# mic-rud/Learned-Compression-of-Point-Cloud-Geometry-and-Attributes

Hardware: AMD Instinct MI355X
Metric: encode+decode Mpoints/sec (higher is better)
Workload: dtype f32

## Files before the change

### include/pcc_hip.h

```cpp
#ifndef PCC_HIP_H
#define PCC_HIP_H

#include <stdint.h>

#ifdef __cplusplus
extern "C" {
#endif

#define PCC_OK 0
#define PCC_ERR_ARG (-1)
#define PCC_ERR_HIP (-2)
#define PCC_ERR_UNSUPPORTED (-3)
#define PCC_ERR_DATA (-4)

#define PCC_ACT_NONE 0
#define PCC_ACT_RELU 1
#define PCC_ACT_LEAKY_RELU 2

int pcc_version(void);
const char* pcc_last_error(void);
int pcc_device_count(void);
int pcc_device_name(int dev, char* out, int out_len);

int64_t pcc_hash_capacity(int64_t n);
// ... 40 lines not shown
int pcc_pair_count(const uint32_t* row_mask, int64_t n_out, int64_t* pair_count, void* stream);

int64_t pcc_order_scratch_bytes(int64_t n);
int pcc_order_rows_by_mask(const uint32_t* row_mask, const int32_t* coords, int64_t n,
                           int32_t block_log2, int32_t tensor_stride, int32_t* order, uint32_t* group_mask32,
                           void* scratch, int64_t scratch_bytes, void* stream);
int pcc_permute_map_rows(const int32_t* nbr, const int32_t* order, int64_t n, int32_t K, int32_t* nbr_sorted, void* stream);

int64_t pcc_small_map_max(void);
int32_t pcc_small_paths(int32_t mask);
int pcc_small_kernel_map(const int32_t* out_coords, int64_t n_out, const uint64_t* in_keys, const int32_t* in_vals, int64_t in_cap,
                         int32_t ksize, int32_t step, int32_t sign, int32_t* nbr, uint32_t* row_mask, int32_t* order,
                         uint32_t* group_mask32, void* scratch, int64_t scratch_bytes, void* stream);

int64_t pcc_conv_packed_elems(int32_t K, int32_t cin, int32_t cout);
int pcc_conv_pack_weights(const float* w, int32_t K, int32_t cin, int32_t cout, float* w_packed,
                          void* stream);
int pcc_conv_fwd(const float* fin, int64_t n_in, int32_t cin, const float* w, const float* w_packed,
                 const float* bias, const int32_t* nbr, const int32_t* order,
                 const uint32_t* group_mask32, int32_t K, float* fout, int64_t n_out, int32_t cout,
                 int32_t act, const float* film, const float* residual, void* stream);

int64_t pcc_conv_small_max(int64_t workgroups);

int pcc_conv_kernel_name(int32_t mode, int64_t n_in, int32_t cin, int32_t cout, int64_t n_out, int32_t K, int32_t has_nbr,
                         char* buf, int32_t len);

int64_t pcc_conv_packed_elems_bf16(int32_t K, int32_t cin, int32_t cout);
int pcc_conv_pack_weights_bf16(const float* w, int32_t K, int32_t cin, int32_t cout, uint16_t* w_packed, void* stream);
int pcc_conv_fwd_bf16(const uint16_t* fin, int64_t n_in, int32_t cin, const uint16_t* w_packed, const float* bias,
                      const int32_t* nbr, const int32_t* order, const uint32_t* group_mask32, int32_t K, float* fout,
                      int64_t n_out, int32_t cout, int32_t act, const float* film, const float* residual, void* stream);

int pcc_epilogue_fwd(const float* c, const float* film, const float* residual, int64_t n, int32_t channels, int32_t act,
                     float* out, void* stream);
int pcc_epilogue_bwd(const float* dout, const float* c, const float* film, int64_t n, int32_t channels, int32_t act,
                     float* dc, float* dfilm, void* stream);

int64_t pcc_cast_colsum_scratch_elems(int32_t channels);
int pcc_cast_colsum(const float* x, int64_t n, int32_t channels, uint16_t* out_bf16, float* colsum, float* scratch,
                    int64_t scratch_elems, void* stream);

int64_t pcc_conv_packed_elems_x3(int32_t K, int32_t cin, int32_t cout);
int pcc_conv_pack_weights_x3(const float* w, int32_t K, int32_t cin, int32_t cout, uint16_t* w_packed, void* stream);
int pcc_conv_fwd_x3(const float* fin, int64_t n_in, int32_t cin, const uint16_t* w_packed, const float* bias,
                    const int32_t* nbr, const int32_t* order, const uint32_t* group_mask32, int32_t K, float* fout,
                    int64_t n_out, int32_t cout, int32_t act, const float* film, const float* residual, void* stream);

int pcc_im2col_thin(const float* fin, int32_t cin, const int32_t* nbr, int64_t n_out, int32_t K, float* out, int32_t k2,
                    void* stream);

int pcc_gather_sum_fwd(const float* scores, int32_t ld, const int32_t* nbr, int32_t K, int32_t cout,
                       const float* bias, float* out, int64_t n_out, int32_t act, void* stream);

int pcc_gather_rows(const float* src, int32_t c, const int32_t* idx, int64_t n, float* out,
                    int32_t accumulate, void* stream);

int pcc_scatter_rows(const float* src, int32_t c, const int32_t* idx, int64_t n, float* out,
                     void* stream);
int pcc_scatter_add_rows(const float* src, int32_t c, const int32_t* idx, int64_t n, float* out,
                         void* stream);

int pcc_compact_rows(const uint8_t* mask, int64_t n, const int32_t* coords, int32_t* out_coords,
                     const float* feats, int32_t c, float* out_feats, int32_t* new_index,
                     int32_t* scratch, int64_t* out_count, void* stream);

int64_t pcc_topk_state_elems(int32_t nbatch);
int pcc_topk_mask(const float* logits, int32_t ld, const int32_t* coords, int64_t n, int32_t nbatch,
                  const int32_t* k, uint8_t* mask, int32_t* state, void* stream);

int pcc_count_per_batch(const int32_t* coords, int64_t n, int32_t nbatch, int32_t* counts, void* stream);

int64_t pcc_sort_scratch_bytes(int64_t n);
int pcc_sort_coords(const int32_t* coords, int64_t n, int32_t* perm, void* scratch,
                    int64_t scratch_bytes, void* stream);

int pcc_kernel_map_transpose(const int32_t* nbr, int64_t n_out, int32_t K, int64_t n_in, int32_t* nbr_t,
                             uint32_t* row_mask_t, void* stream);
int64_t pcc_conv_wgrad_scratch_elems(int32_t K, int32_t cin, int32_t cout);
int pcc_conv_wgrad(const float* fin, int64_t n_in, int32_t cin, const float* dy, int64_t n_out, int32_t cout,
                   const int32_t* nbr, const int32_t* order, const uint32_t* group_mask32, int32_t K, float* dw,
                   float* scratch, int64_t scratch_elems, void* stream);
int pcc_conv_wgrad_kernel_name(int32_t bf16, int32_t K, int32_t cin, int32_t cout, int64_t n_out, char* buf, int32_t len,
                               int32_t* split, int32_t* partials);
int pcc_conv_wgrad_bf16(const uint16_t* fin, int64_t n_in, int32_t cin, const uint16_t* dy, int64_t n_out, int32_t cout,
                        const int32_t* nbr, const int32_t* order, const uint32_t* group_mask32, int32_t K, float* dw,
                        float* scratch, int64_t scratch_elems, void* stream);

int pcc_chconv(const float* x, int64_t n, int32_t c, const int32_t* coords, const uint64_t* keys, const int32_t* vals,
               int64_t cap, int32_t tensor_stride, int32_t ksize, const float* w, int32_t w_channels, int32_t flip,
               float* y, void* stream);

int64_t pcc_octree_scratch_bytes(int64_t n);
int pcc_octree_occupancy(const int32_t* coords, int64_t n, int32_t stride, const int32_t* origin,
                         int32_t depth, uint8_t* occupancy, int32_t* level_counts, void* scratch,
                         int64_t scratch_bytes, void* stream);
int pcc_octree_expand(const uint8_t* occupancy, const int64_t* level_counts, int32_t depth,
                      int32_t stride, const int32_t* origin, int32_t batch, int64_t n_points,
                      int32_t* coords_out, void* scratch, int64_t scratch_bytes, void* stream);

int pcc_octree_context_levels(const int32_t* coords, int64_t n, int32_t stride, const int32_t* origin,
                              int32_t depth, uint8_t* occupancy, uint8_t* patterns, uint32_t* hists,
                              int32_t* level_counts, void* scratch, int64_t scratch_bytes, void* stream);
int pcc_octree_patterns(const uint64_t* nodes, int64_t n, int32_t level, uint8_t* patterns, void* stream);
int pcc_octree_expand_level(const uint64_t* nodes, const uint8_t* occupancy, int64_t n, int64_t n_next,
                            uint64_t* next, void* scratch, int64_t scratch_bytes, void* stream);
// ... 121 lines not shown
```

### learned-compression-of-point-cloud-geometry-and-attributes_amd/_build.py

```python
import os
import subprocess

_HERE = os.path.dirname(os.path.abspath(__file__))
SO_PATH = os.path.join(_HERE, "libpcc_hip.so")

NO_SCRATCH = {
    "conv": ("conv_small_kernel", "conv_mfma_buf_kernel", "conv_mfma_kernel"),
    "rans_lanes": ("rans_lanes_encode_kernel", "rans_lanes_pack_kernel", "rans_lanes_decode_kernel"),
    "chconv": ("chconv_kernel",),
    "augment": ("jitter_partial_kernel", "jitter_mean_kernel", "jitter_apply_kernel", "first_rows_clear_kernel",
                "first_rows_insert_kernel", "first_rows_flag_kernel", "first_rows_finalize_kernel"),
    "normals": ("estimate_normals_kernel",),
    "voxelize": ("first_rows_clear_kernel", "first_rows_insert_kernel", "first_rows_flag_kernel", "first_rows_finalize_kernel",
                 "voxelize_accumulate_kernel"),
    "raht": ("raht_plan_kernel", "raht_step_kernel", "raht_fold_kernel"),
    "pcqm": ("surface_variation_kernel", "pcqm_features_kernel"),
    "render": ("splat_kernel", "gather_kernel"),
}


def build(force=False):
    args = ["make", "-s", "-C", os.path.join(_HERE, "csrc"), "-j4"]
    if force:
        subprocess.check_call(args + ["clean"])
    subprocess.check_call(args)
    for stem, kernels in NO_SCRATCH.items():
        check_kernel_resources(os.path.join(_HERE, "build", stem + ".resources.txt"), kernels)
    check_small_kernel_lds_reads()
    return SO_PATH


def check_small_kernel_lds_reads(obj=None):
    import glob
    import shutil
    objdump = "/opt/rocm/lib/llvm/bin/llvm-objdump"
    obj = obj or os.path.join(_HERE, "build", "conv.o")
    if not os.path.exists(objdump) or not os.path.exists(obj):
        raise RuntimeError(f"cannot lint conv_small_kernel: {objdump} or {obj} is missing")
    tmp = os.path.join(_HERE, "build", "_lint")
    shutil.rmtree(tmp, ignore_errors=True)
    os.makedirs(tmp)
    local = os.path.join(tmp, "conv.o")
    shutil.copy(obj, local)
    subprocess.run([objdump, "--offloading", local], check=True, capture_output=True, cwd=tmp)
    cos = [f for f in glob.glob(local + ".*") if "amdgcn" in f]
    if not cos:
        raise RuntimeError("cannot lint conv_small_kernel: no device code object in build/conv.o")
    dis = subprocess.run([objdump, "-d", cos[0]], check=True, capture_output=True, text=True).stdout
    shutil.rmtree(tmp, ignore_errors=True)
    return lint_lds_reads(dis)


def lint_lds_reads(dis, kernel="conv_small_kernel"):
    import re

    def regs(operand):
        m = re.fullmatch(r"v\[(\d+):(\d+)\]", operand)
        if m:
            return set(range(int(m.group(1)), int(m.group(2)) + 1))
        m = re.fullmatch(r"v(\d+)", operand)
# ... 67 lines not shown
```

### learned-compression-of-point-cloud-geometry-and-attributes_amd/csrc/conv.hip

```cpp
#include <stdlib.h>

#include <type_traits>

#include "common.h"

namespace pcc {

typedef float f32x2 __attribute__((ext_vector_type(2)));
typedef float f32x4 __attribute__((ext_vector_type(4)));
typedef __bf16 bf16x8 __attribute__((ext_vector_type(8)));

struct ConvArgs {
    const float* fin;
    const float* w;
    const float* wp;
    const float* bias;
    const int32_t* nbr;
    const int32_t* order;
    const uint32_t* gmask;
    float* fout;
    const float* film;
    const float* residual;
    int64_t n_in, n_out;
    int cin, cout, coutp, K, act;
// ... 305 lines not shown
        for_live_pattern<MT>(live_tiles(mmask, k), [&](auto live_tag) {
            mfma_step<decltype(live_tag)::value, BN, false>(acc, a_addr, w_addr);
        });
    };

    if (tmask != 0u) {
        uint32_t rem = tmask;
        int k = __builtin_ctz(rem);
        rem &= rem - 1u;
        int knext = rem ? __builtin_ctz(rem) : -1;
        load_idx(k, idx_cur);
        set_a_src(idx_cur);
        dma_step(k, 0, 0);
        load_idx(knext >= 0 ? knext : k, idx_nxt);
        __syncthreads();
        int c = 0, cur = 0;
        while (true) {
            int nk = k, nc = c + 1;
            if (nc == CCH) { nc = 0; nk = knext; }
            const bool has_next = nk >= 0;
            const bool advance = (nc == 0);
            if (advance) {
#pragma unroll
                for (int i = 0; i < RPT; ++i) idx_cur[i] = idx_nxt[i];
                set_a_src(idx_cur);
            }
            if (has_next) {
                dma_step(nk, nc, cur ^ 1);
            }
            uint32_t rem2 = rem;
            int kn2 = knext;
            if (advance) { rem2 &= rem2 - 1u; kn2 = rem2 ? __builtin_ctz(rem2) : -1; }
            load_idx(kn2 >= 0 ? kn2 : k, idx_nxt);
            compute(cur, k);
            __syncthreads();
            if (!has_next) break;
            if (advance) { k = nk; rem = rem2; knext = kn2; }
            c = nc;
            cur ^= 1;
        }
    }

    conv_store_tiles(a, acc, row0 + wrow, nt * BN + wcol + r, h);
}

template <int I, int N, class F>
__device__ __forceinline__ void static_for(F&& f) {
    if constexpr (I < N) {
        f(std::integral_constant<int, I>{});
        static_for<I + 1, N>(f);
    }
}

template <int BM, int BN, int WAVES_M, int WAVES_N, int CCH, bool HAS_NBR, bool BF16 = false, bool X3 = false>
__global__ __launch_bounds__(256) void conv_mfma_buf_kernel(const ConvArgs a) {
#if defined(__HIP_DEVICE_COMPILE__)
    constexpr int RPT = BM / 32;
    constexpr int WM = BM / WAVES_M, WN = BN / WAVES_N;
    constexpr int MT = WM / 32, NT = WN / 32;
    constexpr int A_ELEMS = BM * 32;
    constexpr int W_ELEMS = (X3 ? 12 : 8) * BN * 4;
    constexpr int W_LOADS = ((X3 ? 12 : 8) * BN) / 256;
    static_assert(WAVES_M * WAVES_N == 4 && MT >= 1 && MT <= 2 && NT >= 1 && W_LOADS >= 1, "bad tiling");
    static_assert(!(BF16 && X3), "one operand mode at a time");
    constexpr int ESZ = BF16 ? 2 : 4;

    extern __shared__ __attribute__((aligned(16))) float smem[];
    float* As = smem;
    float* Ws = smem + 2 * A_ELEMS;

    const int t = threadIdx.x;
    const int lane = t & 63, wid = t >> 6;
    const int r = lane & 31, h = lane >> 5;
    const int wrow = (wid / WAVES_N) * WM, wcol = (wid % WAVES_N) * WN;

    const int ntiles_n = a.coutp / BN;
    const int64_t tile = blockIdx.x / ntiles_n;
    const int nt = blockIdx.x - (int)(tile * ntiles_n);
    const int64_t row0 = tile * BM;
    const int K = a.K;

    uint32_t mmask[MT];
    const uint32_t tmask = conv_live_offsets<BM>(a, row0, wrow, mmask);

    f32x16 acc[MT][NT] = {};

    if (tmask != 0u) {
        __amdgpu_buffer_rsrc_t rsrc_a = __builtin_amdgcn_make_buffer_rsrc(
            const_cast<float*>(a.fin), 0, (int)(uint32_t)(a.n_in * a.cin * ESZ), BUF_FLAGS);
        __amdgpu_buffer_rsrc_t rsrc_w = __builtin_amdgcn_make_buffer_rsrc(
            const_cast<float*>(a.wp), 0, (int)((uint32_t)K * a.cin * a.coutp * (X3 ? 6 : ESZ)), BUF_FLAGS);
        __amdgpu_buffer_rsrc_t rsrc_n = __builtin_amdgcn_make_buffer_rsrc(
            const_cast<int32_t*>(a.nbr), 0, HAS_NBR ? (int)(uint32_t)(a.n_out * K * 4) : 0, BUF_FLAGS);

        const int gchunk = t & 7;
        uint32_t q16[RPT], n_voff[RPT], a_voff[RPT];
        int idx_nxt[RPT];
        bool rvalid[RPT];
#pragma unroll
        for (int i = 0; i < RPT; ++i) {
            const int grow = wid * (BM / 4) + 8 * i + (lane >> 3);
            const int64_t pos = row0 + grow;
            rvalid[i] = pos < a.n_out;
            const int64_t ps = rvalid[i] ? pos : a.n_out - 1;
            q16[i] = (uint32_t)((gchunk ^ ((grow >> 1) & 7)) * 16);
            n_voff[i] = (uint32_t)(((HAS_NBR && a.order) ? (int64_t)a.order[ps] : ps) * K * 4);
            idx_nxt[i] = (int)ps;
        }
// ... 107 lines not shown
                PCC_X3_TERM(ah, bh);
#undef PCC_X3_TERM
            }
            __builtin_amdgcn_s_setprio(0);
        };
        auto compute = [&](auto bufc, unsigned live) {
            for_live_pattern<MT>(live, [&](auto live_tag) {
                if constexpr (X3) compute_live_x3(bufc, live_tag);
                else mfma_step<decltype(live_tag)::value, BN, BF16>(acc, a_addr[decltype(bufc)::value], w_addr[decltype(bufc)::value]);
            });
        };

        uint32_t rem = tmask;
        int k = __builtin_ctz(rem);
        rem &= rem - 1u;
        auto offset_body = [&](auto pc) {
            constexpr int P = decltype(pc)::value;
            const int knext = rem ? __builtin_ctz(rem) : -1;
            const uint32_t rem2 = rem & (rem - 1u);
            const int kn2 = rem2 ? __builtin_ctz(rem2) : (knext >= 0 ? knext : k);
            const unsigned live = live_tiles(mmask, k);
            static_for<0, CCH>([&](auto cc) {
                constexpr int c = decltype(cc)::value;
                constexpr int buf = (P + c) & 1;
                if constexpr (c + 1 < CCH) {
                    dma(k, std::integral_constant<int, c + 1>{}, std::integral_constant<int, buf ^ 1>{});
                } else {
                    set_src(knext >= 0);
                    dma(knext >= 0 ? knext : k, std::integral_constant<int, 0>{}, std::integral_constant<int, buf ^ 1>{});
                    load_idx(kn2);
                }
                compute(std::integral_constant<int, buf>{}, live);
                __syncthreads();
            });
            const bool more = knext >= 0;
            k = more ? knext : k;
            rem = rem2;
            return more;
        };

        load_idx(k);
        set_src(true);
        dma(k, std::integral_constant<int, 0>{}, std::integral_constant<int, 0>{});
        load_idx(rem ? __builtin_ctz(rem) : k);
        __syncthreads();
        while (true) {
            if (!offset_body(std::integral_constant<int, 0>{})) break;
            if constexpr (CCH & 1) {
                if (!offset_body(std::integral_constant<int, 1>{})) break;
            }
        }
    }

    conv_store_tiles(a, acc, row0 + wrow, nt * BN + wcol + r, h);
#endif
}

template <int SC, int NS>
constexpr int conv_small_lds_bytes() { return (NS * SC * (32 * 32 + 8 * 32 * 4) + 32 * 32) * (int)sizeof(float); }

template <int SC, int NS>
__global__ __launch_bounds__(512) void conv_small_kernel(const ConvArgs a) {
#if defined(__HIP_DEVICE_COMPILE__)
    constexpr int A_STAGE = SC * 32 * 32;
    constexpr int W_STAGE = SC * 8 * 32 * 4;
    constexpr int STAGE = A_STAGE + W_STAGE;
    constexpr int DMAS = 2 * SC;
    static_assert(NS >= 2 && (NS - 1) * DMAS <= 63, "vmcnt is a 6-bit counter");
    extern __shared__ __attribute__((aligned(16))) float smem[];
    int* idx_s = reinterpret_cast<int*>(smem + NS * STAGE);

    const int t = threadIdx.x;
    const int lane = t & 63;
    const int wave_u = __builtin_amdgcn_readfirstlane(t >> 6);
    const int K = a.K;
    const int ntiles_n = a.coutp / 32;
    const int64_t tile = blockIdx.x / ntiles_n;
    const int nt = blockIdx.x - (int)(tile * ntiles_n);
    const int64_t row0 = tile * 32;
    uint32_t tmask = (K >= 32) ? 0xffffffffu : ((1u << K) - 1u);
    if (a.gmask) tmask &= a.gmask[row0 >> 5];
    tmask = __builtin_amdgcn_readfirstlane(tmask);
    const int CG = (a.cin / 32) / SC;
    const int total = __builtin_popcount(tmask) * CG;
    constexpr int WAIT_FIRST = (NS - 1) * DMAS, WAIT_LOOP = (NS - 2) * DMAS;

    if (tmask != 0u) {
        for (int e = t; e < 32 * K; e += 512) {
            const int lr = e / K;
            const int64_t pos = row0 + lr;
            idx_s[e] = pos < a.n_out ? a.nbr[(a.order ? (int64_t)a.order[pos] : pos) * K + (e - lr * K)] : -1;
        }
        __syncthreads();
    }
    if (wave_u >= 4) {
        if (tmask == 0u) return;
        const int lw = wave_u - 4, tl = t - 256;
        __amdgpu_buffer_rsrc_t rsrc_a = __builtin_amdgcn_make_buffer_rsrc(const_cast<float*>(a.fin), 0, (int)(uint32_t)(a.n_in * a.cin * 4), BUF_FLAGS);
        __amdgpu_buffer_rsrc_t rsrc_w = __builtin_amdgcn_make_buffer_rsrc(const_cast<float*>(a.wp), 0, (int)((uint32_t)K * a.cin * a.coutp * 4), BUF_FLAGS);
        const int grow = 8 * lw + (lane >> 3);
        const uint32_t q16 = (uint32_t)(((tl & 7) ^ ((grow >> 1) & 7)) * 16);
        const uint32_t w_voff = (uint32_t)(((tl >> 5) * a.coutp + nt * 32 + (tl & 31)) * 16);
        const uint32_t w_kstride = (uint32_t)(a.cin / 4) * a.coutp * 16;
        const uint32_t w_cstride = 8u * a.coutp * 16;
        const uint32_t a_row_bytes = (uint32_t)a.cin * 4;
        uint32_t rem_i = tmask;
        int k_i = __builtin_ctz(rem_i), cg_i = 0, issued = 0, st_i = 0;
        rem_i &= rem_i - 1u;
// ... 294 lines not shown
static int check_shape(const ConvArgs& a, ConvMode mode, const char* who) {
    PCC_REQUIRE(a.K >= 1 && a.K <= 27, "%s: K=%d out of range", who, a.K);
    if (mode == CONV_F32) PCC_REQUIRE(a.cin % 32 != 0 || a.cin <= 256, "%s: MFMA path supports cin <= 256 (got %d)", who, a.cin);
    if (mode == CONV_BF16) PCC_REQUIRE(a.cin % 64 == 0 && a.cin <= 256, "%s: cin must be a multiple of 64 up to 256 (got %d)", who, a.cin);
    if (mode == CONV_X3) PCC_REQUIRE(a.cin % 32 == 0 && a.cin <= 256, "%s: cin must be a multiple of 32 up to 256 (got %d)", who, a.cin);
    PCC_REQUIRE(a.nbr != nullptr || (a.K == 1 && a.n_in == a.n_out), "%s: nbr == NULL needs K == 1 and n_in == n_out", who);
    return PCC_OK;
}

static int plan_conv(const ConvArgs& a, ConvMode mode, ConvPlan& p, const char* who) {
    p = ConvPlan{};
    if (mode == CONV_F32 && a.cin % 32 != 0) {
        if (!thin_cin(a.cin)) {
            pcc::set_error("%s: unsupported cin=%d (need a multiple of 32 or one of 1,2,3,4,6,8,12,16,24)", who, a.cin);
            return PCC_ERR_UNSUPPORTED;
        }
        const size_t lds = (size_t)a.K * a.cin * a.cout * sizeof(float);
        PCC_REQUIRE(lds <= 160 * 1024, "conv(thin): weights %zu B exceed the 160 KB of LDS (cin=%d cout=%d K=%d)", lds, a.cin, a.cout, a.K);
        p.family = FAM_THIN;
        p.cpt = (a.cout % 8 == 0) ? 8 : (a.cout % 4 == 0) ? 4 : (a.cout % 2 == 0) ? 2 : 1;
        return PCC_OK;
    }
    const bool wide = a.coutp % 128 == 0;
    p.family = FAM_BUF;
    p.cch = a.cin / (mode == CONV_BF16 ? 64 : 32);
    if (mode == CONV_F32) {
        const bool buffer = conv_path() == 0 && fits_buffer_path(a);
        const int64_t wgs32 = ((a.n_out + 31) / 32) * (a.coutp / 32);
        if (a.nbr && buffer && wgs32 <= small_max_value() * (wide ? 1 : 2)) {
            p.family = FAM_SMALL;
            p.sc = (p.cch % 4 == 0 && wgs32 <= 256) ? 4 : p.cch % 2 == 0 ? 2 : 1;
            p.ns = p.sc == 1 ? 8 : 3;
            return PCC_OK;
        }
        if (!buffer) p.family = FAM_GLOBAL;
    } else if (mode == CONV_BF16) {
        PCC_REQUIRE((uint64_t)a.n_in * a.cin * 2 <= BUF_OOB && (uint64_t)a.n_out * a.K * 4 <= BUF_OOB,
                    "%s: operands of 4 GiB and more are not supported", who);
    } else {
        PCC_REQUIRE((uint64_t)a.n_in * a.cin * 4 <= BUF_OOB && (uint64_t)a.n_out * a.K * 4 <= BUF_OOB &&
                    (uint64_t)a.K * a.cin * a.coutp * 6 <= BUF_OOB, "%s: operands of 4 GiB and more are not supported", who);
    }
    const int64_t wgs128 = ((a.n_out + 63) / 64) * (a.coutp / 128);
    auto tile = [&](int bm, int bn, int wm, int wn) { p.bm = bm; p.bn = bn; p.wm = wm; p.wn = wn; return PCC_OK; };
    if (wide && wgs128 < FILL_WGS) return tile(64, 64, 2, 2);
    if (wide && mode == CONV_F32 && wgs128 < ROW32_MAX_WGS) return tile(32, 128, 1, 4);
    if (wide) return tile(64, 128, 2, 2);
    if (a.coutp % 64 == 0) return mode == CONV_X3 ? tile(64, 64, 2, 2) : tile(128, 64, 2, 2);
    if (mode != CONV_X3) return tile(128, 32, 4, 1);
    pcc::set_error("%s: cout=%d not supported (output width rounded up to 32 must be a multiple of 64)", who, a.cout);
    return PCC_ERR_UNSUPPORTED;
}

template <auto KERN>
static int launch(int64_t blocks, int threads, size_t lds, size_t lds_limit, const ConvArgs& a, hipStream_t st) {
    static bool limit_set = false;
    if (lds_limit && !limit_set) {
        PCC_CHECK_HIP(hipFuncSetAttribute(reinterpret_cast<const void*>(KERN), hipFuncAttributeMaxDynamicSharedMemorySize, (int)lds_limit));
        limit_set = true;
    }
    PCC_REQUIRE(blocks < (1ll << 31), "conv: grid too large");
    hipLaunchKernelGGL(KERN, dim3((unsigned)blocks), dim3(threads), lds, st, a);
    PCC_LAUNCH_CHECK();
    return PCC_OK;
}

template <ConvMode M, int BM, int BN, int WM, int WN, int CCH>
static int launch_buf(int64_t blocks, const ConvArgs& a, hipStream_t st) {
    constexpr bool BF16 = M == CONV_BF16, X3 = M == CONV_X3;
    if constexpr (BF16 && CCH > 4) {
        return PCC_ERR_UNSUPPORTED;
    } else {
        constexpr int lds = conv_lds_bytes<BM, BN, X3>();
        return a.nbr ? launch<conv_mfma_buf_kernel<BM, BN, WM, WN, CCH, true, BF16, X3>>(blocks, 256, lds, lds, a, st)
                     : launch<conv_mfma_buf_kernel<BM, BN, WM, WN, CCH, false, BF16, X3>>(blocks, 256, lds, lds, a, st);
    }
}

template <ConvMode M, int BM, int BN, int WM, int WN>
static int launch_mfma(const ConvPlan& p, const ConvArgs& a, hipStream_t st) {
    const int64_t blocks = (a.n_out + BM - 1) / BM * (a.coutp / BN);
    if constexpr (M == CONV_F32) {
        if (p.family == FAM_GLOBAL) {
            constexpr int lds = conv_lds_bytes<BM, BN>();
            return a.nbr ? launch<conv_mfma_kernel<BM, BN, WM, WN, true>>(blocks, 256, lds, lds, a, st)
                         : launch<conv_mfma_kernel<BM, BN, WM, WN, false>>(blocks, 256, lds, lds, a, st);
        }
    }
    switch (p.cch) {
        case 1: return launch_buf<M, BM, BN, WM, WN, 1>(blocks, a, st);
        case 2: return launch_buf<M, BM, BN, WM, WN, 2>(blocks, a, st);
        case 3: return launch_buf<M, BM, BN, WM, WN, 3>(blocks, a, st);
        case 4: return launch_buf<M, BM, BN, WM, WN, 4>(blocks, a, st);
        case 5: return launch_buf<M, BM, BN, WM, WN, 5>(blocks, a, st);
        case 6: return launch_buf<M, BM, BN, WM, WN, 6>(blocks, a, st);
        case 7: return launch_buf<M, BM, BN, WM, WN, 7>(blocks, a, st);
        case 8: return launch_buf<M, BM, BN, WM, WN, 8>(blocks, a, st);
        default: return PCC_ERR_UNSUPPORTED;
    }
}

template <ConvMode M>
static int launch_tile(const ConvPlan& p, const ConvArgs& a, hipStream_t st) {
    if (p.bm == 64 && p.bn == 64) return launch_mfma<M, 64, 64, 2, 2>(p, a, st);
    if (p.bm == 64 && p.bn == 128) return launch_mfma<M, 64, 128, 2, 2>(p, a, st);
    if constexpr (M == CONV_F32)
        if (p.bm == 32) return launch_mfma<M, 32, 128, 1, 4>(p, a, st);
    if constexpr (M != CONV_X3) {
// ... 11 lines not shown

template <int CIN>
static int launch_thin(const ConvPlan& p, const ConvArgs& a, hipStream_t st) {
    const size_t lds = (size_t)a.K * CIN * a.cout * sizeof(float);
    const unsigned nb = blocks_for(a.n_out * (a.cout / p.cpt), 256, lds >= 4096 ? 2048u : (1u << 20));
    const size_t limit = lds > 64 * 1024 ? 160 * 1024 : 0;
    if (p.cpt == 8) return launch<conv_thin_kernel<CIN, 8>>(nb, 256, lds, limit, a, st);
    if (p.cpt == 4) return launch<conv_thin_kernel<CIN, 4>>(nb, 256, lds, limit, a, st);
    if (p.cpt == 2) return launch<conv_thin_kernel<CIN, 2>>(nb, 256, lds, limit, a, st);
    return launch<conv_thin_kernel<CIN, 1>>(nb, 256, lds, limit, a, st);
}

static int launch_thin_cin(const ConvPlan& p, const ConvArgs& a, hipStream_t st) {
    switch (a.cin) {
        case 1: return launch_thin<1>(p, a, st);
        case 2: return launch_thin<2>(p, a, st);
        case 3: return launch_thin<3>(p, a, st);
        case 4: return launch_thin<4>(p, a, st);
        case 6: return launch_thin<6>(p, a, st);
        case 8: return launch_thin<8>(p, a, st);
        case 12: return launch_thin<12>(p, a, st);
        case 16: return launch_thin<16>(p, a, st);
        case 24: return launch_thin<24>(p, a, st);
        default: return PCC_ERR_UNSUPPORTED;
    }
}

static int conv_fwd(ConvMode mode, const ConvArgs& a, void* stream) {
    const char* who = CONV_ENTRY[mode];
    int rc = check_shape(a, mode, who);
    if (rc != PCC_OK) return rc;
    PCC_REQUIRE(a.act >= 0 && a.act <= 2, "%s: bad activation %d", who, a.act);
    if (mode == CONV_F32 && a.n_out <= 0) return PCC_OK;
    if (mode != CONV_F32 || a.cin % 32 == 0) {
        PCC_REQUIRE(a.wp != nullptr, "%s: MFMA path (cin=%d) needs packed weights", who, a.cin);
        PCC_REQUIRE(((reinterpret_cast<uintptr_t>(a.fin) | reinterpret_cast<uintptr_t>(a.wp)) & 15) == 0,
                    "%s: fin and w_packed must be 16-byte aligned (16-byte LDS-DMA loads)", who);
    } else {
        PCC_REQUIRE(a.w != nullptr, "%s: thin path (cin=%d) needs raw weights", who, a.cin);
    }
    if (a.n_out <= 0) return PCC_OK;
    ConvPlan p;
    if ((rc = plan_conv(a, mode, p, who)) != PCC_OK) return rc;
    hipStream_t st = as_stream(stream);
    switch (p.family) {
        case FAM_THIN: return launch_thin_cin(p, a, st);
        case FAM_SMALL:
            if (p.sc == 4) return launch_small<4, 3>(a, st);
            return p.sc == 2 ? launch_small<2, 3>(a, st) : launch_small<1, 8>(a, st);
        default:
            if (mode == CONV_BF16) return launch_tile<CONV_BF16>(p, a, st);
            return mode == CONV_X3 ? launch_tile<CONV_X3>(p, a, st) : launch_tile<CONV_F32>(p, a, st);
    }
}

template <class T>
static int pack_weights(const char* who, void (*kern)(const float*, int, int, int, int, int, T*), int cin_pad, const float* w,
                        int K, int cin, int cout, T* w_packed, void* stream) {
    PCC_REQUIRE(K >= 1 && cin >= 1 && cout >= 1, "%s: bad shape", who);
    const int cinp = (cin + cin_pad - 1) / cin_pad * cin_pad, coutp = round_up32(cout);
    const int64_t total = (int64_t)K * cinp * coutp;
    hipLaunchKernelGGL(kern, dim3(blocks_for(total, 256, 4096)), dim3(256), 0, as_stream(stream), w, K, cin, cout, cinp, coutp,
                       w_packed);
    PCC_LAUNCH_CHECK();
    return PCC_OK;
}

}

using namespace pcc;

extern "C" {

int64_t pcc_conv_packed_elems(int32_t K, int32_t cin, int32_t cout) {
    return (int64_t)K * round_up32(cin) * round_up32(cout);
}

int pcc_conv_pack_weights(const float* w, int32_t K, int32_t cin, int32_t cout, float* w_packed, void* stream) {
    return pack_weights("pcc_conv_pack_weights", pack_weights_kernel, 32, w, K, cin, cout, w_packed, stream);
}

int64_t pcc_conv_packed_elems_bf16(int32_t K, int32_t cin, int32_t cout) {
    return (int64_t)K * ((cin + 63) / 64 * 64) * round_up32(cout);
}

int pcc_conv_pack_weights_bf16(const float* w, int32_t K, int32_t cin, int32_t cout, uint16_t* w_packed, void* stream) {
    return pack_weights("pcc_conv_pack_weights_bf16", pack_weights_bf16_kernel, 64, w, K, cin, cout,
                        reinterpret_cast<__bf16*>(w_packed), stream);
}

int pcc_conv_fwd_bf16(const uint16_t* fin, int64_t n_in, int32_t cin, const uint16_t* w_packed, const float* bias, const int32_t* nbr,
                      const int32_t* order, const uint32_t* group_mask32, int32_t K, float* fout, int64_t n_out, int32_t cout,
                      int32_t act, const float* film, const float* residual, void* stream) {
    return conv_fwd(CONV_BF16, {reinterpret_cast<const float*>(fin), nullptr, reinterpret_cast<const float*>(w_packed), bias, nbr, order,
                                group_mask32, fout, film, residual, n_in, n_out, cin, cout, round_up32(cout), K, act}, stream);
}

int64_t pcc_conv_packed_elems_x3(int32_t K, int32_t cin, int32_t cout) {
    return (int64_t)K * round_up32(cin) * round_up32(cout) * 3;
}

int pcc_conv_pack_weights_x3(const float* w, int32_t K, int32_t cin, int32_t cout, uint16_t* w_packed, void* stream) {
    return pack_weights("pcc_conv_pack_weights_x3", pack_weights_x3_kernel, 32, w, K, cin, cout, w_packed, stream);
}

int pcc_conv_fwd_x3(const float* fin, int64_t n_in, int32_t cin, const uint16_t* w_packed, const float* bias, const int32_t* nbr,
                    const int32_t* order, const uint32_t* group_mask32, int32_t K, float* fout, int64_t n_out, int32_t cout,
                    int32_t act, const float* film, const float* residual, void* stream) {
    return conv_fwd(CONV_X3, {fin, nullptr, reinterpret_cast<const float*>(w_packed), bias, nbr, order, group_mask32, fout, film,
                              residual, n_in, n_out, cin, cout, round_up32(cout), K, act}, stream);
}

int pcc_im2col_thin(const float* fin, int32_t cin, const int32_t* nbr, int64_t n_out, int32_t K, float* out, int32_t k2,
                    void* stream) {
    PCC_REQUIRE(K >= 1 && K <= 27 && cin >= 1 && cin <= 16, "pcc_im2col_thin: bad shape (K=%d cin=%d)", K, cin);
    PCC_REQUIRE(k2 % 32 == 0 && k2 >= K * cin, "pcc_im2col_thin: row length %d must be a multiple of 32 and >= K * cin = %d", k2, K * cin);
    PCC_REQUIRE(nbr != nullptr && (reinterpret_cast<uintptr_t>(out) & 15) == 0, "pcc_im2col_thin: nbr required, out 16-byte aligned");
    if (n_out <= 0) return PCC_OK;
    hipLaunchKernelGGL(im2col_thin_kernel, dim3(blocks_for(n_out * (k2 / 4), 256, 1 << 20)), dim3(256), 0, as_stream(stream), fin, cin, nbr,
                       n_out, K, out, k2);
    PCC_LAUNCH_CHECK();
    return PCC_OK;
}

int pcc_gather_sum_fwd(const float* scores, int32_t ld, const int32_t* nbr, int32_t K, int32_t cout, const float* bias,
                       float* out, int64_t n_out, int32_t act, void* stream) {
    PCC_REQUIRE(K >= 1 && K <= 27 && cout >= 1 && ld >= K * cout, "pcc_gather_sum_fwd: bad shape (K=%d cout=%d ld=%d)", K, cout, ld);
    PCC_REQUIRE(nbr != nullptr, "pcc_gather_sum_fwd: neighbour table required");
    PCC_REQUIRE(act >= 0 && act <= 2, "pcc_gather_sum_fwd: bad activation %d", act);
    if (n_out <= 0) return PCC_OK;
    const unsigned nb27 = blocks_for(n_out, 256);
    const bool al16 = (reinterpret_cast<uintptr_t>(nbr) & 15) == 0;
#define PCC_GS27(C)                                                                                                    \
    hipLaunchKernelGGL(gather_sum27_kernel<C>, dim3(nb27), dim3(256), 0, as_stream(stream), scores, ld, nbr, bias, out, n_out, act)
    if (K == 27 && al16 && cout == 1) PCC_GS27(1);
    else if (K == 27 && al16 && cout == 2) PCC_GS27(2);
    else if (K == 27 && al16 && cout == 3) PCC_GS27(3);
    else if (K == 27 && al16 && cout == 4) PCC_GS27(4);
    else
#undef PCC_GS27
        hipLaunchKernelGGL(gather_sum_kernel, dim3(blocks_for(n_out * cout, 256, 1 << 20)), dim3(256), 0, as_stream(stream),
                           scores, ld, nbr, K, cout, bias, out, n_out, act);
    PCC_LAUNCH_CHECK();
    return PCC_OK;
}

int64_t pcc_conv_small_max(int64_t workgroups) {
    const int64_t before = small_max_value();
    if (workgroups >= 0) g_small_max = workgroups;
    return before;
}

int pcc_conv_fwd(const float* fin, int64_t n_in, int32_t cin, const float* w, const float* w_packed, const float* bias,
                 const int32_t* nbr, const int32_t* order, const uint32_t* group_mask32, int32_t K, float* fout,
                 int64_t n_out, int32_t cout, int32_t act, const float* film, const float* residual, void* stream) {
    return conv_fwd(CONV_F32, {fin, w, w_packed, bias, nbr, order, group_mask32, fout, film, residual, n_in, n_out, cin, cout,
                               round_up32(cout), K, act}, stream);
}

int pcc_conv_kernel_name(int32_t mode, int64_t n_in, int32_t cin, int32_t cout, int64_t n_out, int32_t K, int32_t has_nbr,
                         char* buf, int32_t len) {
    PCC_REQUIRE(mode >= CONV_F32 && mode <= CONV_X3, "pcc_conv_kernel_name: bad mode %d", mode);
    static const int32_t any_map = 0;
    ConvArgs a = {};
    a.nbr = has_nbr ? &any_map : nullptr;
    a.n_in = n_in; a.n_out = n_out; a.cin = cin; a.cout = cout; a.coutp = round_up32(cout); a.K = K;
    const ConvMode m = ConvMode(mode);
    ConvPlan p;
    if (check_shape(a, m, CONV_ENTRY[m]) != PCC_OK || plan_conv(a, m, p, CONV_ENTRY[m]) != PCC_OK) return PCC_ERR_UNSUPPORTED;
    if (buf == nullptr) return PCC_OK;
    const char* tf = has_nbr ? "true" : "false";
    int n;
    if (p.family == FAM_THIN) n = snprintf(buf, len, "conv_thin_kernel<%d, %d>", cin, p.cpt);
    else if (p.family == FAM_SMALL) n = snprintf(buf, len, "conv_small_kernel<%d, %d>", p.sc, p.ns);
    else if (p.family == FAM_GLOBAL) n = snprintf(buf, len, "conv_mfma_kernel<%d, %d, %d, %d, %s>", p.bm, p.bn, p.wm, p.wn, tf);
    else n = snprintf(buf, len, "conv_mfma_buf_kernel%s<%d, %d, %d, %d, %d, %s>", CONV_TAG[m], p.bm, p.bn, p.wm, p.wn, p.cch, tf);
    PCC_REQUIRE(n < len, "pcc_conv_kernel_name: %d bytes do not hold the name", len);
    return PCC_OK;
}

}
```

### learned-compression-of-point-cloud-geometry-and-attributes_amd/sparse.py

```python
import ctypes
import functools
import math
import weakref

import os

import torch
import torch.nn as nn

from . import _lib, _threads
from ._lib import PCC, check, ptr

ACT_NONE, ACT_RELU, ACT_LRELU = PCC.ACT_NONE, PCC.ACT_RELU, PCC.ACT_LEAKY_RELU


def _require_cuda(t):
    if not t.is_cuda:
        raise RuntimeError("libpcc_hip operators need tensors on an MI355X device (got a CPU tensor); "
                           "there is no CPU fallback")


COORD_PROFILER = None


# ... 544 lines not shown
    return ev


def _prof_end(ev0, name, cin, cout, pairs, n_out, gmask=None):
    if PROFILER is None:
        return
    ev1 = None
    if ev0 is not None:
        ev1 = torch.cuda.Event(enable_timing=True)
        ev1.record()
    PROFILER.append((name, cin, cout, pairs, n_out, ev0, ev1, gmask))


_MFMA_VISIT = (0, 4, 1, 5, 2, 6, 3, 7)


def _thin_im2col_forward(x_feats, in_map, out_map, layer, ksize, transposed, act, film, residual, out_channels):
    L = _lib.lib()
    w2p, bias, k2, cout = layer.im2col_weights(out_channels)
    nbr, _, pairs = in_map.kernel_map(out_map, ksize, transposed)
    n_out, K, cin = out_map.n, ksize ** 3, x_feats.shape[1]
    dev = x_feats.device
    x2 = torch.empty((n_out, k2), dtype=torch.float32, device=dev)
    out = torch.empty((n_out, cout), dtype=torch.float32, device=dev)
    ev0 = _prof_begin()
    ev = _cp_begin()
    check(L.pcc_im2col_thin(ptr(x_feats), cin, ptr(nbr), n_out, K, ptr(x2), k2, _lib.stream()))
    _cp_end(ev, "im2col_thin", n_out, lambda: 4 * K * n_out + 4 * cin * int(pairs) + 4 * k2 * n_out)
    check(L.pcc_conv_fwd(ptr(x2), n_out, k2, None, ptr(w2p), ptr(bias), None, None, None, 1, ptr(out), n_out, cout, act, ptr(film),
                         ptr(residual), _lib.stream()))
    _prof_end(ev0, f"thin_im2col<{cin}>", cin, cout, pairs, n_out)
    return out


def _narrow_head_forward(x_feats, in_map, out_map, layer, ksize, transposed, act, out_channels):
    L = _lib.lib()
    w_r, wp_r, bias, K, cout = layer.narrow_weights(out_channels)
    n_in, cin = x_feats.shape
    n_out = out_map.n
    nbr, _, pairs = in_map.kernel_map(out_map, ksize, transposed)
    ld = K * cout
    scores = torch.empty((n_in, ld), dtype=torch.float32, device=x_feats.device)
    out = torch.empty((n_out, cout), dtype=torch.float32, device=x_feats.device)
    ev0 = _prof_begin()
    check(L.pcc_conv_fwd(ptr(x_feats), n_in, cin, ptr(w_r), ptr(wp_r), None, None, None, None, 1, ptr(scores), n_in, ld,
                         ACT_NONE, None, None, _lib.stream()))
    ev = _cp_begin()
    check(L.pcc_gather_sum_fwd(ptr(scores), ld, ptr(nbr), K, cout, ptr(bias), ptr(out), n_out, act, _lib.stream()))
    _cp_end(ev, "gather_sum", n_out, lambda: 4 * K * n_out + 4 * cout * int(pairs) + 4 * cout * n_out)
    _prof_end(ev0, f"narrow_head<{cin}>", cin, cout, pairs, n_out)
    return out


def set_conv_small_max(workgroups):
    return int(_lib.lib().pcc_conv_small_max(int(workgroups)))


NARROW_HEAD_MAX_COUT = 4

CHECK_EXPECTED_COUNTS = os.environ.get("PCC_CHECK_COUNTS", "0") == "1"
ORDER_BLOCK_LOG2 = int(os.environ.get("PCC_ORDER_BLOCK_LOG2", "-1"))

INFER_BF16 = os.environ.get("PCC_INFER_BF16", "0") == "1"


def set_infer_bf16(enabled):
    global INFER_BF16
    INFER_BF16 = bool(enabled)


INFER_X3 = os.environ.get("PCC_INFER_X3", "0") == "1"


def set_infer_x3(enabled):
    global INFER_X3
    INFER_X3 = bool(enabled)


GATE_LOG = None


PROFILER = None
PROFILER_MIN_ROWS = 65536


MODE_F32, MODE_BF16, MODE_X3 = 0, 1, 2


def conv_kernel_name(mode, n_in, cin, cout, n_out, K, has_nbr):
    buf = ctypes.create_string_buffer(128)
    check(_lib.lib().pcc_conv_kernel_name(mode, n_in, cin, cout, n_out, K, int(has_nbr), buf, len(buf)))
    return buf.value.decode()


def launch_mode(bf16, x3, n_in, cin, cout, n_out, K, has_nbr):
    if bf16 and _plan_takes(MODE_BF16, n_in, cin, cout, n_out, K, has_nbr):
        return MODE_BF16
    if x3 and _plan_takes(MODE_X3, n_in, cin, cout, n_out, K, has_nbr):
        return MODE_X3
    return MODE_F32


@functools.lru_cache(maxsize=4096)
def _plan_takes(mode, n_in, cin, cout, n_out, K, has_nbr):
    return _lib.lib().pcc_conv_kernel_name(mode, n_in, cin, cout, n_out, K, int(has_nbr), None, 0) == 0

# ... 166 lines not shown
        self.kernel = nn.Parameter(torch.empty((self.kernel_size ** 3, self.in_channels), dtype=torch.float32))
        bound = 1.0 / math.sqrt(self.kernel_size ** 3)
        with torch.no_grad():
            self.kernel.uniform_(-bound, bound)

    def forward(self, x):
        from .autograd import ChannelwiseConvFn, chconv_launch
        kernel = self.kernel
        c = x.F.shape[1]
        if kernel.dim() != 2 or kernel.shape[0] != self.kernel_size ** 3 or kernel.shape[1] not in (1, c):
            raise ValueError(f"kernel of shape {tuple(kernel.shape)} on {c} channels: need [{self.kernel_size ** 3}, 1 or {c}]")
        _require_cuda(kernel)
        if torch.is_grad_enabled() and kernel.requires_grad:
            raise NotImplementedError("MinkowskiChannelwiseConvolution: the kernel's gradient is not built; "
                                      "set kernel.requires_grad = False")
        window = kernel.detach().to(torch.float32).contiguous()
        if _tracked(x.F):
            feats = ChannelwiseConvFn.apply(x.F, window, x.map, self.kernel_size)
        else:
            feats = chconv_launch(x.F.contiguous(), x.map, window, self.kernel_size, 0)
        return SparseTensor._wrap(feats, x.map)


class MinkowskiReLU(nn.Module):
    act = ACT_RELU

    def __init__(self, inplace=False):
        super().__init__()


class MinkowskiLeakyReLU(MinkowskiReLU):
    act = ACT_LRELU


class ConvChain(nn.Sequential):

    def plan(self):
        hit = self.__dict__.get("_plan")
        if hit is not None and hit[0] == len(self):
            return hit[1]
        steps = []
        mods = list(self)
        i = 0
        while i < len(mods):
            m = mods[i]
            assert isinstance(m, _ConvBase), f"unexpected module {type(m)} at {i}"
            act = ACT_NONE
            if i + 1 < len(mods) and isinstance(mods[i + 1], MinkowskiReLU):
                act = mods[i + 1].act
                i += 1
            steps.append((m, act))
            i += 1
        self.__dict__["_plan"] = (len(self), steps)
        return steps

    def forward(self, x, last_film=None, last_residual=None, last_out_map=None, last_out_channels=None):
        steps = self.plan()
        last_j = len(steps) - 1
        for j, (m, act) in enumerate(steps):
            if j == last_j:
                x = m.forward(x, act, last_film, last_residual, last_out_map, last_out_channels)
            else:
                x = m.forward(x, act)
        return x


class MinkowskiPruning(nn.Module):

    def forward(self, x, mask):
        coords, feats, _, _ = compact_rows(mask.to(torch.uint8), x.C, x.F)
        return SparseTensor(feats, coordinate_map=CoordMap(coords, x.map.stride, nbatch=x.map._nbatch))
```

Measured before the change: 9.084.

## Fuse hidden sparse conv with narrow head score GEMM in one kernel

Adds a conv_head_buf_kernel that runs the hidden layer's MFMA sparse convolution and, instead of storing its activations, writes the bias plus activation result into LDS. It then multiplies that tile by the narrow head's packed weights to produce per-offset scores directly. The Python Sequential forward detects a trailing hidden conv + ReLU + narrow head pair and routes inference through the fused path, followed by the existing gather_sum. This removes the hidden activation round trip through global memory and one kernel launch. In exchange it adds LDS reuse constraints and a restricted set of supported shapes.

```diff
diff --git a/include/pcc_hip.h b/include/pcc_hip.h
--- a/include/pcc_hip.h
+++ b/include/pcc_hip.h
@@ -116,6 +116,11 @@
 
 int pcc_gather_sum_fwd(const float* scores, int32_t ld, const int32_t* nbr, int32_t K, int32_t cout,
                        const float* bias, float* out, int64_t n_out, int32_t act, void* stream);
+
+int pcc_conv_head_supported(int64_t n_in, int32_t cin, int32_t cout, int64_t n_out, int32_t K, int32_t head_cols);
+int pcc_conv_head_fwd(const float* fin, int64_t n_in, int32_t cin, const float* w_packed, const float* bias, const int32_t* nbr,
+                      const int32_t* order, const uint32_t* group_mask32, int32_t K, int64_t n_out, int32_t cout, int32_t act,
+                      const float* head_w_packed, int32_t head_cols, float* scores, void* stream);
 
 int pcc_gather_rows(const float* src, int32_t c, const int32_t* idx, int64_t n, float* out,
                     int32_t accumulate, void* stream);
diff --git a/learned-compression-of-point-cloud-geometry-and-attributes_amd/_build.py b/learned-compression-of-point-cloud-geometry-and-attributes_amd/_build.py
--- a/learned-compression-of-point-cloud-geometry-and-attributes_amd/_build.py
+++ b/learned-compression-of-point-cloud-geometry-and-attributes_amd/_build.py
@@ -5,7 +5,7 @@
 SO_PATH = os.path.join(_HERE, "libpcc_hip.so")
 
 NO_SCRATCH = {
-    "conv": ("conv_small_kernel", "conv_mfma_buf_kernel", "conv_mfma_kernel"),
+    "conv": ("conv_small_kernel", "conv_mfma_buf_kernel", "conv_mfma_kernel", "conv_head_buf_kernel"),
     "rans_lanes": ("rans_lanes_encode_kernel", "rans_lanes_pack_kernel", "rans_lanes_decode_kernel"),
     "chconv": ("chconv_kernel",),
     "augment": ("jitter_partial_kernel", "jitter_mean_kernel", "jitter_apply_kernel", "first_rows_clear_kernel",
diff --git a/learned-compression-of-point-cloud-geometry-and-attributes_amd/csrc/conv.hip b/learned-compression-of-point-cloud-geometry-and-attributes_amd/csrc/conv.hip
--- a/learned-compression-of-point-cloud-geometry-and-attributes_amd/csrc/conv.hip
+++ b/learned-compression-of-point-cloud-geometry-and-attributes_amd/csrc/conv.hip
@@ -381,8 +381,8 @@
     }
 }
 
-template <int BM, int BN, int WAVES_M, int WAVES_N, int CCH, bool HAS_NBR, bool BF16 = false, bool X3 = false>
-__global__ __launch_bounds__(256) void conv_mfma_buf_kernel(const ConvArgs a) {
+template <int BM, int BN, int WAVES_M, int WAVES_N, int CCH, bool HAS_NBR, bool BF16, bool X3, class Epilogue>
+__device__ __forceinline__ void conv_buf_tile(const ConvArgs& a, Epilogue&& epilogue) {
 #if defined(__HIP_DEVICE_COMPILE__)
     constexpr int RPT = BM / 32;
     constexpr int WM = BM / WAVES_M, WN = BN / WAVES_N;
@@ -596,8 +596,102 @@
         }
     }
 
-    conv_store_tiles(a, acc, row0 + wrow, nt * BN + wcol + r, h);
+    epilogue(acc, row0, nt);
 #endif
+}
+
+template <int BM, int BN, int WAVES_M, int WAVES_N, int CCH, bool HAS_NBR, bool BF16 = false, bool X3 = false>
+__global__ __launch_bounds__(256) void conv_mfma_buf_kernel(const ConvArgs a) {
+    conv_buf_tile<BM, BN, WAVES_M, WAVES_N, CCH, HAS_NBR, BF16, X3>(a, [&](const auto& acc, int64_t row0, int nt) {
+        const int lane = threadIdx.x & 63, wid = threadIdx.x >> 6;
+        conv_store_tiles(a, acc, row0 + (wid / WAVES_N) * (BM / WAVES_M), nt * BN + (wid % WAVES_N) * (BN / WAVES_N) + (lane & 31), lane >> 5);
+    });
+}
+
+struct ConvHeadArgs {
+    ConvArgs a;
+    const float* wps;
+    float* scores;
+    int sld, sp;
+};
+
+template <int BM, int BN, int WAVES_M, int WAVES_N>
+__device__ __forceinline__ void conv_head_scores(const ConvHeadArgs& ha, const f32x16 (&acc)[BM / WAVES_M / 32][BN / WAVES_N / 32],
+                                                 int64_t row0) {
+#if defined(__HIP_DEVICE_COMPILE__)
+    constexpr int WM = BM / WAVES_M, WN = BN / WAVES_N;
+    constexpr int MT = WM / 32, NT = WN / 32;
+    constexpr int SCH = BN / 32;
+    constexpr int IMG = BM * A_LD_DMA;
+    constexpr int W_OFF = SCH * IMG;
+    static_assert((W_OFF + SCH * 1024) * (int)sizeof(float) <= conv_lds_bytes<BM, BN>(), "images and slabs exceed the main loop's LDS");
+    const ConvArgs& a = ha.a;
+    extern __shared__ __attribute__((aligned(16))) float smem[];
+
+    const int t = threadIdx.x;
+    const int lane = t & 63, wid = t >> 6;
+    const int r = lane & 31, h = lane >> 5;
+    const int wrow = (wid / WAVES_N) * WM, wcol = (wid % WAVES_N) * WN;
+
+    const int wave_u = __builtin_amdgcn_readfirstlane(wid);
+    __amdgpu_buffer_rsrc_t rsrc_s = __builtin_amdgcn_make_buffer_rsrc(const_cast<float*>(ha.wps), 0, (int)((uint32_t)BN * ha.sp * 4), BUF_FLAGS);
+    const uint32_t s_voff = (uint32_t)(((t >> 5) * ha.sp + (t & 31)) * 16);
+    const uint32_t s_cstride = 8u * ha.sp * 16;
+    auto dma_slabs = [&](int n) {
+#pragma unroll
+        for (int c = 0; c < SCH; ++c)
+            __builtin_amdgcn_raw_ptr_buffer_load_lds(rsrc_s, (lds_ptr_t)(smem + W_OFF + c * 1024 + wave_u * 256), 16,
+                                                     s_voff + (uint32_t)n * 512u, (uint32_t)c * s_cstride, 0, 0);
+    };
+    dma_slabs(0);
+
+#pragma unroll
+    for (int m = 0; m < MT; ++m) {
+#pragma unroll
+        for (int n = 0; n < NT; ++n) {
+            const int col = wcol + 32 * n + r;
+            const float bcol = conv_bias(a, col);
+            float* img = smem + ((wcol >> 5) + n) * IMG;
+#pragma unroll
+            for (int reg = 0; reg < 16; ++reg) {
+                const int R = wrow + 32 * m + 4 * h + mfma32_row(reg);
+                img[R * A_LD_DMA + ((((r >> 2) ^ ((R >> 1) & 7))) << 2) + (r & 3)] = apply_act(acc[m][n][reg] + bcol, a.act);
+            }
+        }
+    }
+
+    uint32_t a_addr[SCH][4], w_addr[SCH];
+#pragma unroll
+    for (int c = 0; c < SCH; ++c) {
+#pragma unroll
+        for (int kk = 0; kk < 4; ++kk) a_addr[c][kk] = (uint32_t)(c * IMG * 4) + a_frag_offset(32 * wave_u + r, h, kk);
+        w_addr[c] = (uint32_t)((W_OFF + c * 1024 + (h * 32 + r) * 4) * 4);
+    }
+    const int nts = ha.sp >> 5;
+    for (int n = 0; n < nts; ++n) {
+        if (n > 0) dma_slabs(n);
+        __syncthreads();
+        if (wave_u < BM / 32) {
+            f32x16 s[1][1] = {};
+            static_for<0, SCH>([&](auto cc) { mfma_step<1u, 32, false, 1, 1>(s, a_addr[decltype(cc)::value], w_addr[decltype(cc)::value]); });
+            const int col = 32 * n + r;
+#pragma unroll
+            for (int reg = 0; reg < 16; ++reg) {
+                const int64_t pos = row0 + 32 * wave_u + 4 * h + mfma32_row(reg);
+                if (pos >= a.n_out) continue;
+                ha.scores[(a.order ? (int64_t)a.order[pos] : pos) * ha.sp + col] = s[0][0][reg] + 0.0f;
+            }
+        }
+        if (n + 1 < nts) __syncthreads();
+    }
+#endif
+}
+
+template <int BM, int BN, int WAVES_M, int WAVES_N, int CCH>
+__global__ __launch_bounds__(256) void conv_head_buf_kernel(const ConvHeadArgs ha) {
+    conv_buf_tile<BM, BN, WAVES_M, WAVES_N, CCH, true, false, false>(ha.a, [&](const auto& acc, int64_t row0, int) {
+        conv_head_scores<BM, BN, WAVES_M, WAVES_N>(ha, acc, row0);
+    });
 }
 
 template <int SC, int NS>
@@ -998,8 +1092,8 @@
     return PCC_ERR_UNSUPPORTED;
 }
 
-template <auto KERN>
-static int launch(int64_t blocks, int threads, size_t lds, size_t lds_limit, const ConvArgs& a, hipStream_t st) {
+template <auto KERN, class Args>
+static int launch(int64_t blocks, int threads, size_t lds, size_t lds_limit, const Args& a, hipStream_t st) {
     static bool limit_set = false;
     if (lds_limit && !limit_set) {
         PCC_CHECK_HIP(hipFuncSetAttribute(reinterpret_cast<const void*>(KERN), hipFuncAttributeMaxDynamicSharedMemorySize, (int)lds_limit));
@@ -1117,6 +1211,51 @@
             if (mode == CONV_BF16) return launch_tile<CONV_BF16>(p, a, st);
             return mode == CONV_X3 ? launch_tile<CONV_X3>(p, a, st) : launch_tile<CONV_F32>(p, a, st);
     }
+}
+
+static bool head_plan(const ConvArgs& a, int head_cols, ConvPlan& p) {
+    if (a.nbr == nullptr || a.cin % 32 != 0 || a.cin > 256 || a.cout != a.coutp || a.K < 1 || a.K > 27 || a.n_out <= 0) return false;
+    if (head_cols < 1 || head_cols > 128) return false;
+    if (plan_conv(a, CONV_F32, p, "pcc_conv_head_fwd") != PCC_OK || p.family != FAM_BUF || p.bn != a.coutp) return false;
+    return (p.bm == 128 && p.bn == 64) || (p.bm == 64 && p.bn == 128) || (p.bm == 32 && p.bn == 128);
+}
+
+template <int BM, int BN, int WM, int WN>
+static int launch_head(int cch, const ConvHeadArgs& ha, hipStream_t st) {
+    const int64_t blocks = (ha.a.n_out + BM - 1) / BM;
+    constexpr int lds = conv_lds_bytes<BM, BN>();
+    switch (cch) {
+        case 1: return launch<conv_head_buf_kernel<BM, BN, WM, WN, 1>>(blocks, 256, lds, lds, ha, st);
+        case 2: return launch<conv_head_buf_kernel<BM, BN, WM, WN, 2>>(blocks, 256, lds, lds, ha, st);
+        case 3: return launch<conv_head_buf_kernel<BM, BN, WM, WN, 3>>(blocks, 256, lds, lds, ha, st);
+        case 4: return launch<conv_head_buf_kernel<BM, BN, WM, WN, 4>>(blocks, 256, lds, lds, ha, st);
+        case 5: return launch<conv_head_buf_kernel<BM, BN, WM, WN, 5>>(blocks, 256, lds, lds, ha, st);
+        case 6: return launch<conv_head_buf_kernel<BM, BN, WM, WN, 6>>(blocks, 256, lds, lds, ha, st);
+        case 7: return launch<conv_head_buf_kernel<BM, BN, WM, WN, 7>>(blocks, 256, lds, lds, ha, st);
+        case 8: return launch<conv_head_buf_kernel<BM, BN, WM, WN, 8>>(blocks, 256, lds, lds, ha, st);
+        default: return PCC_ERR_UNSUPPORTED;
+    }
+}
+
+static int conv_head_fwd(const ConvHeadArgs& ha, void* stream) {
+    const ConvArgs& a = ha.a;
+    const char* who = "pcc_conv_head_fwd";
+    int rc = check_shape(a, CONV_F32, who);
+    if (rc != PCC_OK) return rc;
+    PCC_REQUIRE(a.act >= 0 && a.act <= 2, "%s: bad activation %d", who, a.act);
+    PCC_REQUIRE(a.wp != nullptr && ha.wps != nullptr && ha.scores != nullptr, "%s: packed weights of both layers and scores required", who);
+    PCC_REQUIRE(((reinterpret_cast<uintptr_t>(a.fin) | reinterpret_cast<uintptr_t>(a.wp) | reinterpret_cast<uintptr_t>(ha.wps)) & 15) == 0,
+                "%s: fin and the packed weights must be 16-byte aligned (16-byte LDS-DMA loads)", who);
+    if (a.n_out <= 0) return PCC_OK;
+    ConvPlan p;
+    if (!head_plan(a, ha.sld, p)) {
+        pcc::set_error("%s: no fused kernel for this shape (cin=%d cout=%d rows=%lld head columns=%d): ask pcc_conv_head_supported first",
+                       who, a.cin, a.cout, (long long)a.n_out, ha.sld);
+        return PCC_ERR_UNSUPPORTED;
+    }
+    hipStream_t st = as_stream(stream);
+    if (p.bm == 128) return launch_head<128, 64, 2, 2>(p.cch, ha, st);
+    return p.bm == 64 ? launch_head<64, 128, 2, 2>(p.cch, ha, st) : launch_head<32, 128, 1, 4>(p.cch, ha, st);
 }
 
 template <class T>
@@ -1223,6 +1362,23 @@
                                round_up32(cout), K, act}, stream);
 }
 
+int pcc_conv_head_supported(int64_t n_in, int32_t cin, int32_t cout, int64_t n_out, int32_t K, int32_t head_cols) {
+    static const int32_t any_map = 0;
+    ConvArgs a = {};
+    a.nbr = &any_map;
+    a.n_in = n_in; a.n_out = n_out; a.cin = cin; a.cout = cout; a.coutp = round_up32(cout); a.K = K;
+    ConvPlan p;
+    return head_plan(a, head_cols, p) ? 1 : 0;
+}
+
+int pcc_conv_head_fwd(const float* fin, int64_t n_in, int32_t cin, const float* w_packed, const float* bias, const int32_t* nbr,
+                      const int32_t* order, const uint32_t* group_mask32, int32_t K, int64_t n_out, int32_t cout, int32_t act,
+                      const float* head_w_packed, int32_t head_cols, float* scores, void* stream) {
+    ConvHeadArgs ha = {{fin, nullptr, w_packed, bias, nbr, order, group_mask32, nullptr, nullptr, nullptr, n_in, n_out, cin, cout,
+                        round_up32(cout), K, act}, head_w_packed, scores, head_cols, round_up32(head_cols)};
+    return conv_head_fwd(ha, stream);
+}
+
 int pcc_conv_kernel_name(int32_t mode, int64_t n_in, int32_t cin, int32_t cout, int64_t n_out, int32_t K, int32_t has_nbr,
                          char* buf, int32_t len) {
     PCC_REQUIRE(mode >= CONV_F32 && mode <= CONV_X3, "pcc_conv_kernel_name: bad mode %d", mode);
diff --git a/learned-compression-of-point-cloud-geometry-and-attributes_amd/sparse.py b/learned-compression-of-point-cloud-geometry-and-attributes_amd/sparse.py
--- a/learned-compression-of-point-cloud-geometry-and-attributes_amd/sparse.py
+++ b/learned-compression-of-point-cloud-geometry-and-attributes_amd/sparse.py
@@ -620,6 +620,59 @@
     return out
 
 
+FUSE_HEADS = os.environ.get("PCC_FUSE_HEADS", "1") != "0"
+
+
+def set_fuse_heads(enabled):
+    global FUSE_HEADS
+    before, FUSE_HEADS = FUSE_HEADS, bool(enabled)
+    return before
+
+
+def _head_pair(hidden, hid_act, head):
+    for m in (hidden, head):
+        if m.transposed or m.stride != 1 or m.kernel_size <= 1:
+            return False
+    return hid_act == ACT_RELU and hidden.out_channels % 32 == 0 and head.in_channels == hidden.out_channels
+
+
+def _fusable_head(x, hidden, head, film, residual, out_map, out_channels):
+    hcout = head.out_channels if out_channels is None else out_channels
+    if not FUSE_HEADS or hcout > NARROW_HEAD_MAX_COUT or INFER_BF16 or INFER_X3 or film is not None or residual is not None:
+        return False
+    if torch.is_grad_enabled() and (hidden.kernel.requires_grad or head.kernel.requires_grad or x.F.requires_grad):
+        return False
+    if out_map is not None and out_map is not x.map:
+        return False
+    n = x.map.n
+    return bool(_lib.lib().pcc_conv_head_supported(n, hidden.in_channels, hidden.out_channels, n, hidden.kernel_size ** 3,
+                                                   head.kernel_size ** 3 * hcout))
+
+
+def _fused_head_forward(x_feats, cmap, hidden, hid_act, head, act, out_channels):
+    L = _lib.lib()
+    _, wp, hbias = hidden.weights()
+    _, wp_r, bias, K, cout = head.narrow_weights(out_channels)
+    n, cin = x_feats.shape
+    ch = hidden.out_channels
+    Kh = hidden.kernel_size ** 3
+    nbr_h, order, gmask, pairs_h = cmap.conv_map(cmap, hidden.kernel_size, False, cin)
+    nbr, _, pairs = cmap.kernel_map(cmap, head.kernel_size, False)
+    ld = (K * cout + 31) // 32 * 32
+    scores = torch.empty((n, ld), dtype=torch.float32, device=x_feats.device)
+    out = torch.empty((n, cout), dtype=torch.float32, device=x_feats.device)
+    ev0 = _prof_begin()
+    check(L.pcc_conv_head_fwd(ptr(x_feats), n, cin, ptr(wp), ptr(hbias), ptr(nbr_h), ptr(order), ptr(gmask), Kh, n, ch, hid_act,
+                              ptr(wp_r), K * cout, ptr(scores), _lib.stream()))
+    _prof_end(ev0, f"conv_head<{ch}>", cin, ch, pairs_h, n, gmask)
+    ev0 = _prof_begin()
+    ev = _cp_begin()
+    check(L.pcc_gather_sum_fwd(ptr(scores), ld, ptr(nbr), K, cout, ptr(bias), ptr(out), n, act, _lib.stream()))
+    _cp_end(ev, "gather_sum", n, lambda: 4 * K * n + 4 * cout * int(pairs) + 4 * cout * n)
+    _prof_end(ev0, f"narrow_head<{ch}>", ch, cout, pairs, n)
+    return out
+
+
 def set_conv_small_max(workgroups):
     return int(_lib.lib().pcc_conv_small_max(int(workgroups)))
 
@@ -892,12 +945,18 @@
             steps.append((m, act))
             i += 1
         self.__dict__["_plan"] = (len(self), steps)
+        self.__dict__["_head_at"] = len(steps) - 2 if len(steps) >= 2 and _head_pair(steps[-2][0], steps[-2][1], steps[-1][0]) else -1
         return steps
 
     def forward(self, x, last_film=None, last_residual=None, last_out_map=None, last_out_channels=None):
         steps = self.plan()
         last_j = len(steps) - 1
         for j, (m, act) in enumerate(steps):
+            if j == self._head_at and _fusable_head(x, m, steps[last_j][0], last_film, last_residual, last_out_map,
+                                                    last_out_channels):
+                head, head_act = steps[last_j]
+                feats = _fused_head_forward(x.F, x.map, m, act, head, head_act, last_out_channels)
+                return SparseTensor._wrap(feats, x.map)
             if j == last_j:
                 x = m.forward(x, act, last_film, last_residual, last_out_map, last_out_channels)
             else:
```

New measurement: 9.053 (median of 2 runs). About the same (-0.3%).
